# cxjyxxme/deep-online-video-stabilization

Hardware: AMD Instinct MI355X
Metric: stabilized frames/sec (720p, before_ch=31) (higher is better)
Workload: dtype f32 (bf16x3 split MFMA, f32 accumulate); 1 GPU; BASELINE.json configs[1]: v2_93 net, 1280x720, 1 stream(s)/GPU, batch=1 per stream, 13-ch stack from a 32-deep ring (lags 1,2,4,8,16,32; --before-ch 31 ignored as in the reference), ResNet-v2-50 regressor + 4x4 multi-grid warp + feedback; one independent stream set per GPU (replicas only); height=720, width=1280, streams_per_gpu=1, refine=1, operand_mode=4, launches_per_frame=64, hip_graph=True

## Files before the change

deep-online-video-stabilization_amd/csrc/conv.h:

```cpp
#pragma once
#include "common.h"

struct ConvArgs {
    const float* x;
    const float* w;
    float* y;
    const float* bias;
    const float* in_scale;
    const float* in_shift;
    const float* residual;
    const float* out_scale;
    const float* out_shift;
    const float* out_floor;
    float* partial;
    int N, H, W, Cin, Ho, Wo, Cout, KH, KW, stride, pad;
    int up;
    int res_H, res_W, res_stride;
    int relu_out;
    int x_ld, res_ld;
    int M, K;
    int splitk, steps_per_split;
    int cin_real;
    unsigned div_hw_mul, div_hw_shift, div_w_mul, div_w_shift;
    int rowrun;
    int in_scale_expected;
    int xcd_swizzle;
};

size_t conv_plan(ConvArgs& a);
struct Prof;
int conv_launch(const ConvArgs& a, hipStream_t st, Prof* prof = nullptr, int bf16_operands = 0, const float* w_img = nullptr,
                bool lowk_ring = false);

enum ConvFamily {
    CONV_IGEMM,
    CONV_RING,
    CONV_RING_KG,
    CONV_RING_PRO,
    CONV_PACKED,
    CONV_PACKED_KG2,
    CONV_ASTAT,
    CONV_PATCH
};
struct ConvRoute {
    int family;
    int tile, bk, nbuf;
    int mode;
    int operand;
    int kg, pro;
    int reduce;
    int prof_kind;
    int astat_bm;
    int patch_cfg;
};
ConvRoute conv_route(const ConvArgs& a, int operand_mode, bool has_image, bool bound, bool lowk_ring = false );
const char* conv_prof_kind_name(int kind);
size_t conv_weight_image_floats(int Cout, int K);
int launch_weight_split_image(const float* w, int Cout, int K, float* img, hipStream_t st);
struct WeightImageTable { long w_off[64], img_off[64], tprefix[65]; int Cout[64], K[64]; int n; };
void weight_image_table_add(WeightImageTable& t, long w_off, long img_off, int Cout, int K);
int launch_weight_split_images(const float* w_base, float* img_base, const WeightImageTable& t, hipStream_t st);
int conv_reduce_launches(const ConvArgs& a, int operand_mode = 0);

struct ConvPair { int m_tower, x_tower_floats ; long dx, dy, dres, dscale; };
bool conv_pair_supported(const ConvArgs& a);
int conv_launch_pair(const ConvArgs& a, const ConvPair& pr, hipStream_t st, Prof* prof = nullptr,
                     const float* w_img = nullptr );

bool conv_b2b_supported(const ConvArgs& c2, const ConvArgs& c3);
int conv_b2b_launch(const ConvArgs& c2, const ConvArgs& c3, hipStream_t st, Prof* prof = nullptr);

static inline void sn_fastdiv_make(unsigned d, unsigned& mul, unsigned& shift) {
    unsigned l = 0;
    while ((1ull << l) < d) ++l;
    mul = (unsigned)((((1ull << l) - d) << 32) / d + 1);
    shift = l;
}
#ifdef __HIPCC__
__device__ __forceinline__ int sn_fastdiv(int n, unsigned mul, unsigned shift) {
    return (int)((__umulhi(mul, (unsigned)n) + (unsigned)n) >> shift);
}
#endif
```

deep-online-video-stabilization_amd/csrc/conv.hip:

```cpp
#include "conv.h"
#include "prof.h"
#include <climits>
#include <cstdio>
#include <cstdlib>
#include <algorithm>
#include <string>
#include <vector>

#include "conv_kernel.h"
#include "conv_ring_kernel.h"
#include "conv_astat_kernel.h"
#include "conv_patch_kernel.h"
#include "conv_b2b_kernel.h"

template <int PAIR>
__device__ __forceinline__ void conv_splitk_reduce_body(const ConvArgs& p, const ConvPair& pr) {
    const size_t q = (size_t)blockIdx.x * 256 + threadIdx.x;
    const int c4n = p.Cout / 4;
    if (q >= (size_t)p.M * c4n) return;
    const int m = (int)(q / c4n);
    const int n = (int)(q - (size_t)m * c4n) * 4;
    const bool t1 = PAIR && m >= pr.m_tower;
    const size_t slab = (size_t)p.M * p.Cout;
    const float* src = p.partial + (size_t)m * p.Cout + n;
    float4 s = *reinterpret_cast<const float4*>(src);
    for (int z = 1; z < p.splitk; ++z) {
        const float4 t = *reinterpret_cast<const float4*>(src + z * slab);
        s.x += t.x; s.y += t.y; s.z += t.z; s.w += t.w;
    }
    if (p.bias != nullptr) {
        const float4 b = *reinterpret_cast<const float4*>(p.bias + n);
        s.x += b.x; s.y += b.y; s.z += b.z; s.w += b.w;
    }
    if (p.residual != nullptr) {
        size_t ri;
        if (p.res_stride == 1 && p.res_H == p.Ho && p.res_W == p.Wo) {
            ri = (size_t)m * p.res_ld + n;
        } else {
            const int img = sn_fastdiv(m, p.div_hw_mul, p.div_hw_shift);
            const int rr = m - img * (p.Ho * p.Wo);
            const int oy = sn_fastdiv(rr, p.div_w_mul, p.div_w_shift), ox = rr - oy * p.Wo;
            ri = (((size_t)img * p.res_H + oy * p.res_stride) * p.res_W + ox * p.res_stride) * p.res_ld + n;
        }
        const float4 t = *reinterpret_cast<const float4*>(p.residual + (t1 ? pr.dres : 0) + ri);
        s.x += t.x; s.y += t.y; s.z += t.z; s.w += t.w;
    }
    if (p.out_scale != nullptr) {
        const float4 a = *reinterpret_cast<const float4*>(p.out_scale + n), b = *reinterpret_cast<const float4*>(p.out_shift + n);
        s.x = __builtin_fmaf(s.x, a.x, b.x); s.y = __builtin_fmaf(s.y, a.y, b.y);
        s.z = __builtin_fmaf(s.z, a.z, b.z); s.w = __builtin_fmaf(s.w, a.w, b.w);
    }
    if (p.out_scale != nullptr && p.out_floor != nullptr) {
        const float4 f = *reinterpret_cast<const float4*>(p.out_floor + n);
        s.x = fmaxf(s.x, f.x); s.y = fmaxf(s.y, f.y); s.z = fmaxf(s.z, f.z); s.w = fmaxf(s.w, f.w);
    } else if (p.relu_out) {
        s.x = fmaxf(s.x, 0.f); s.y = fmaxf(s.y, 0.f); s.z = fmaxf(s.z, 0.f); s.w = fmaxf(s.w, 0.f);
    }
    *reinterpret_cast<float4*>(p.y + (t1 ? pr.dy : 0) + (size_t)m * p.Cout + n) = s;
}
__global__ __launch_bounds__(256) void conv_splitk_reduce_kernel(const ConvArgs p) {
    conv_splitk_reduce_body<0>(p, ConvPair{});
}
__global__ __launch_bounds__(256) void conv_splitk_reduce_pair_kernel(const ConvArgs p, const ConvPair pr) {
    conv_splitk_reduce_body<1>(p, pr);
}

enum TileId { T128x128 = 0, T128x64 = 1, T64x64 = 2 };

static void tile_dims(int t, int& bm, int& bn) {
    bm = (t == T64x64) ? 64 : 128;
    bn = (t == T128x128) ? 128 : 64;
}

static int env_int(const char* name, int dflt) {
    const char* v = getenv(name);
    return v ? atoi(v) : dflt;
}

struct ConvSwitches {
    int tile = env_int("STABNET_CONV_TILE", -1), splitk = env_int("STABNET_CONV_SPLITK", -1);
    int bk16 = env_int("STABNET_CONV_BK16", 0);
    int nbuf = env_int("STABNET_CONV_NBUF", 0);
    int tuning_table = env_int("STABNET_CONV_TUNING_TABLE", 1);
    int split_below = env_int("STABNET_CONV_SPLIT_BELOW", 400), split_target = env_int("STABNET_CONV_SPLIT_TARGET", 448);
    int xcd = env_int("STABNET_CONV_XCD", 1);
    int ring = env_int("STABNET_CONV_RING", 1), ring_wgs_per_cu = env_int("STABNET_CONV_RING_WGS_PER_CU", 3);
    int lowk_igemm = env_int("STABNET_CONV_LOWK_IGEMM", 1);
    int ring_pro = env_int("STABNET_CONV_RING_PRO", 1);
    int kgroups = env_int("STABNET_CONV_KGROUPS", 1), kgroups_pro = env_int("STABNET_CONV_KGROUPS_PRO", 1);
    int packed_kg2 = env_int("STABNET_CONV_PACKED_KG2", 1), packed_kg3 = env_int("STABNET_CONV_PACKED_KG3", 1);
    int packed_pro = env_int("STABNET_CONV_PACKED_PRO", 1);
    int packed_wgs_per_cu = env_int("STABNET_CONV_PACKED_WGS_PER_CU", 2);
    int astat = env_int("STABNET_CONV_ASTAT", 1), astat_min_m = env_int("STABNET_CONV_ASTAT_MIN_M", 0);
    int astat_min_cout = env_int("STABNET_CONV_ASTAT_MIN_COUT", 256);
    int patch = env_int("STABNET_CONV_PATCH", 1), patch_min_m = env_int("STABNET_CONV_PATCH_MIN_M", 0);
    int patch_cfg = env_int("STABNET_CONV_PATCH_CFG", 0);
    int b2b = env_int("STABNET_CONV_B2B", 1), b2b_wgs_per_cu = env_int("STABNET_CONV_B2B_WGS_PER_CU", 2);
};
static const ConvSwitches& sw() {
    static const ConvSwitches s;
    return s;
}

static int g_force_tile = -2, g_force_split = -1;
static int force_tile() { return g_force_tile == -2 ? sw().tile : g_force_tile; }
static int force_split() { return g_force_tile == -2 ? sw().splitk : g_force_split; }

static int conv_bk(const ConvArgs& a) { return (a.rowrun || (a.Cin % 32 == 0 && !sw().bk16)) ? 32 : 16; }
static int conv_total_steps(const ConvArgs& a) {
    if (a.rowrun) return a.KH * cdiv(a.KW * a.Cin, 32);
    return a.KH * a.KW * (a.Cin / conv_bk(a));
}

struct TuneEntry { int M, Cout, K, KH, ring, splitk; };
#include "conv_tuning_table.h"
#include "conv_tuning_table_packed.h"
static int g_tuning_profile = 0;
static std::vector<TuneEntry> g_tuning_runtime;

static int tuning_lookup(int M, int Cout, int K, int KH, int ring) {
    for (const TuneEntry& e : g_tuning_runtime)
        if (e.M == M && e.Cout == Cout && e.K == K && e.KH == KH && e.ring == ring) return e.splitk;
    if (sw().tuning_table && g_tuning_profile == 1)
        for (const TuneEntry& e : g_tuning_packed)
            if (e.M == M && e.Cout == Cout && e.K == K && e.KH == KH && e.ring == ring) return e.splitk;
    if (sw().tuning_table)
        for (const TuneEntry& e : g_tuning_builtin)
            if (e.M == M && e.Cout == Cout && e.K == K && e.KH == KH && e.ring == ring) return e.splitk;
    return 0;
}

static int pick_tile(const ConvArgs& a, int& splitk) {
    if (force_tile() >= 0) {
        const int steps0 = conv_total_steps(a);
        splitk = force_split() > 0 ? std::min(force_split(), steps0) : 1;
        return force_tile();
    }
    const int total_steps = conv_total_steps(a);
    const long blocks = (long)cdiv(a.M, 64) * cdiv(a.Cout, 64);
    const bool ring_path = a.rowrun || (a.in_scale_expected == 0 && a.up == 1 && a.Cin % 32 == 0);
    int s = tuning_lookup(a.M, a.Cout, a.K, a.KH, ring_path ? 1 : 0);
    const int thr = sw().split_below, target = sw().split_target;
    if (s > 0) {
        s = std::min(s, std::max(1, total_steps / 2));
    } else if (blocks < thr && a.Cout % 4 == 0) {
        s = (int)((target + blocks / 2) / blocks);
        s = std::min(s, std::max(1, total_steps / 8));
        s = std::min(s, 32);
    } else {
        s = 1;
    }
    splitk = std::max(1, s);
    return T64x64;
}

size_t conv_plan(ConvArgs& a) {
    a.xcd_swizzle = sw().xcd;
    a.M = a.N * a.Ho * a.Wo;
    a.K = a.rowrun ? a.KH * 32 * cdiv(a.KW * a.Cin, 32) : a.KH * a.KW * a.Cin;
    if (a.x_ld == 0) a.x_ld = a.Cin;
    if (a.res_ld == 0) a.res_ld = a.Cout;
    sn_fastdiv_make((unsigned)(a.Ho * a.Wo), a.div_hw_mul, a.div_hw_shift);
    sn_fastdiv_make((unsigned)a.Wo, a.div_w_mul, a.div_w_shift);
    int splitk = 1;
    (void)pick_tile(a, splitk);
    const int total_steps = conv_total_steps(a);
    a.steps_per_split = cdiv(total_steps, splitk);
    a.splitk = cdiv(total_steps, a.steps_per_split);
    return a.splitk > 1 ? (size_t)a.splitk * a.M * a.Cout * sizeof(float) : 0;
}

static void igemm_variant(const ConvArgs& a, int bm, int bn, int bk, int mode, int operand, int& nbuf_out, int& bf16_out) {
    const int nbuf = sw().nbuf;
    bf16_out = (bm == 64 && bn == 64 && bk == 32) ? operand : 0;
    const bool one_stage = nbuf == 1 || (nbuf == 0 && mode == 0 && bm == 64 && bn == 64 && a.M >= 32768);
    nbuf_out = (bf16_out != 1 && one_stage) ? 1 : 2;
}

static bool ring_eligible(const ConvArgs& a, int tile, bool has_prologue, bool lowk_ring = false) {
    if (a.rowrun) return true;
    if (!lowk_ring && sw().lowk_igemm && a.KH == 1 && a.KW == 1 && a.Cin == 64 && a.x_ld == a.Cin && a.out_floor == nullptr) return false;
    return sw().ring && tile == T64x64 && !has_prologue && a.up == 1 && a.Cin % 32 == 0 && !sw().bk16;
}

static bool ring_pro_vectors_ok(const ConvArgs& a) {
    if (a.in_scale == nullptr || a.in_shift == nullptr) return true;
    const long d = (long)(a.in_shift - a.in_scale);
    return d >= 0 && d < (1L << 30);
}
static bool ring_pro_geometry(const ConvArgs& a, int operand, bool has_prologue) {
    return sw().ring_pro && sw().ring && operand != 1 && !sw().bk16 && has_prologue && a.KH == 1 && a.KW == 1 && a.stride == 1 && a.pad == 0 &&
           a.up == 1 && a.Cin % 32 == 0 && !a.rowrun && a.x_ld == a.Cin;
}
static bool ring_pro_eligible(const ConvArgs& a, int operand) {
    return ring_pro_geometry(a, operand, a.in_scale != nullptr) && a.out_scale == nullptr && a.out_floor == nullptr && ring_pro_vectors_ok(a);
}

static int conv_kgroups(const ConvArgs& a, int operand, bool ring, bool has_prologue) {
    if (!sw().kgroups || a.splitk < 2 || operand == 1) return 1;
    if (a.steps_per_split * a.splitk != conv_total_steps(a)) return 1;
    if (ring && a.splitk == 3 && !a.rowrun) return 3;
    if (sw().kgroups_pro && !ring && a.splitk == 2 && ring_pro_geometry(a, operand, has_prologue) && ring_pro_vectors_ok(a)) return 2;
    return 1;
}

struct PatchForm { int ph, pw, wr, ns; };
static const PatchForm g_patch_forms[] = {{8, 8, 1, 3}, {8, 8, 2, 3}};
constexpr int SN_PATCH_FORMS = 2;
constexpr size_t SN_PATCH_LDS_MAX = 160 * 1024;
static int patch_cfg(const ConvArgs& a) {
    auto fits = [&](int cfg) { return sn_patch_lds_bytes(g_patch_forms[cfg - 1].ph, g_patch_forms[cfg - 1].pw, a.Cin) <= SN_PATCH_LDS_MAX; };
    const int forced = sw().patch_cfg;
    if (forced >= 1 && forced <= SN_PATCH_FORMS) return fits(forced) ? forced : 0;
    const int cfg = a.Cout <= 64 ? 1 : 2;
    return fits(cfg) ? cfg : 0;
}

static int route_prof_kind(const ConvRoute& r) {
    switch (r.family) {
        case CONV_IGEMM:
            return PK_KERNEL_CONV_BASE + r.mode * 6 + r.tile * 2 + (r.bk == 32 ? 1 : 0) + (r.nbuf == 1 ? 18 : 0) + 36 * r.operand;
        case CONV_PACKED: return PK_KERNEL_CONV_PACKED + (r.pro ? 3 : r.mode);
        case CONV_PACKED_KG2: return PK_KERNEL_CONV_PACKED + (r.pro ? 6 : 4 + r.mode);
        case CONV_ASTAT: return PK_KERNEL_CONV_ASTAT;
        case CONV_PATCH: return PK_KERNEL_CONV_PATCH + r.patch_cfg - 1;
        default: break;
    }
    const int split = r.operand >= 2 ? PK_KERNEL_CONV_SPLIT + 8 * (r.operand - 2) : 0;
    if (r.family == CONV_RING) return split ? split + r.mode : PK_KERNEL_CONV_RING + r.mode + (r.operand ? 3 : 0);
    if (r.family == CONV_RING_PRO) return split ? split + 5 : PK_KERNEL_CONV_KG + 2;
    if (r.kg == 2) return split ? split + 6 : PK_KERNEL_CONV_KG + 3;
    return split ? split + 3 + r.mode : PK_KERNEL_CONV_KG + r.mode;
}

ConvRoute conv_route(const ConvArgs& a, int operand_mode, bool has_image, bool bound, bool lowk_ring) {
    const ConvSwitches& s = sw();
    const bool image = operand_mode == 4 && has_image;
    const int op = operand_mode == 4 ? 0 : operand_mode;
    int splitk_unused = 1;
    const int t = pick_tile(a, splitk_unused);
    const bool t64 = t == T64x64, bk32 = conv_bk(a) == 32;
    const bool has_pro = bound ? a.in_scale != nullptr : a.in_scale_expected != 0;
    const bool ring = ring_eligible(a, t, has_pro, lowk_ring && image);
    const bool slabs = !bound || a.splitk == 1 || a.partial != nullptr;
    int kg = t64 ? conv_kgroups(a, op, ring, has_pro) : 1;
    if (image && s.packed_kg3 && ring && kg == 3 && a.K % 32 == 0 && slabs) kg = 1;
    const bool pro = kg == 1 && !ring && t64 && bk32 && (bound ? ring_pro_eligible(a, op) : ring_pro_geometry(a, op, has_pro));
    const bool packed_pro = image && s.packed_pro && !ring && t64 && bk32 && ring_pro_geometry(a, op, has_pro) &&
                            (!bound || a.out_floor == nullptr)  && ring_pro_vectors_ok(a) && slabs;
    if (packed_pro) kg = 1;
    const bool packed = (image && ring && kg == 1 && a.K % 32 == 0) || packed_pro;
    const bool packed_kg2 = packed && s.packed_kg2 && a.splitk == 2 && !a.rowrun && a.steps_per_split * 2 == conv_total_steps(a);
    if (packed_kg2) kg = 2;
    const int astat_min_m = s.astat_min_m > 0 ? s.astat_min_m : ((long)a.Cout * a.K >= 128 * 1024 ? 2048 : 8192);
    const bool astat = packed && !packed_pro && !packed_kg2 && kg == 1 && a.splitk == 1 && s.astat && !lowk_ring && !a.rowrun &&
                       a.KH == 1 && a.KW == 1 && a.stride == 1 && a.pad == 0 && a.up == 1 && a.K <= 256 && a.Cout >= s.astat_min_cout &&
                       a.M >= astat_min_m;
    const int patch_form = patch_cfg(a);
    const bool patch = packed && !packed_pro && ((kg == 1 && a.splitk == 1) || packed_kg2) && s.patch && !lowk_ring && !a.rowrun &&
                       a.KH == 3 && a.KW == 3 && a.stride == 1 && a.pad == 1 && a.up == 1 && a.Cin % 32 == 0 && patch_form != 0 &&
                       a.M >= (s.patch_min_m > 0 ? s.patch_min_m : 12288);

    ConvRoute r{};
    r.tile = t;
    r.bk = bk32 ? 32 : 16;
    r.mode = (a.up > 1 || a.rowrun) ? 2 : (a.pad == 0 ? 0 : 1);
    r.operand = op;
    r.kg = kg;
    r.reduce = (a.splitk > 1 && kg == 1) ? 1 : 0;
    if (astat) {
        r.family = CONV_ASTAT;
        r.operand = 4;
        r.astat_bm = 32;
    } else if (patch) {
        r.family = CONV_PATCH;
        r.operand = 4;
        r.patch_cfg = patch_form;
    } else if (packed) {
        r.family = packed_kg2 ? CONV_PACKED_KG2 : CONV_PACKED;
        r.operand = 4;
        r.pro = packed_pro ? 1 : 0;
    } else if (pro) {
        r.family = CONV_RING_PRO;
        r.pro = 1;
    } else if (kg > 1) {
        r.family = CONV_RING_KG;
        r.pro = kg == 2 ? 1 : 0;
    } else if (ring) {
        r.family = CONV_RING;
    } else {
        int bm, bn;
        tile_dims(t, bm, bn);
        r.family = CONV_IGEMM;
        igemm_variant(a, bm, bn, r.bk, r.mode, op, r.nbuf, r.operand);
    }
    r.prof_kind = route_prof_kind(r);
    return r;
}

int conv_reduce_launches(const ConvArgs& a, int operand_mode) {
    return a.splitk < 2 ? 0 : conv_route(a, operand_mode, operand_mode == 4, false).reduce;
}

const char* conv_prof_kind_name(int kind) {
    static const std::vector<std::string> names = [] {
        std::vector<std::string> v(PK_KERNEL_CONV_BASE + 144);
        char buf[96];
        auto ring = [&](int family, int mode, int operand, int kg, int pro) {
            ConvRoute r{};
            r.family = family; r.mode = mode; r.operand = operand; r.kg = kg; r.pro = pro;
            snprintf(buf, sizeof(buf), "conv_ring_f32_kernel<%d, %d, %d, %d>", mode, operand, kg, pro);
            v[route_prof_kind(r)] = buf;
        };
        for (int operand = 0; operand < 4; ++operand) {
            for (int mode = 0; mode < 3; ++mode) ring(CONV_RING, mode, operand, 1, 0);
            if (operand == 1) continue;
            ring(CONV_RING_KG, 0, operand, 3, 0); ring(CONV_RING_KG, 1, operand, 3, 0);
            ring(CONV_RING_PRO, 0, operand, 1, 1); ring(CONV_RING_KG, 0, operand, 2, 1);
        }
        for (int mode = 0; mode < 3; ++mode) ring(CONV_PACKED, mode, 4, 1, 0);
        ring(CONV_PACKED, 0, 4, 1, 1);
        ring(CONV_PACKED_KG2, 0, 4, 2, 0); ring(CONV_PACKED_KG2, 1, 4, 2, 0); ring(CONV_PACKED_KG2, 0, 4, 2, 1);
        {
            ConvRoute r{};
            r.family = CONV_ASTAT; r.astat_bm = 32;
            snprintf(buf, sizeof(buf), "conv_astat_f32_kernel<%d>", r.astat_bm);
            v[route_prof_kind(r)] = buf;
        }
        for (int cfg = 1; cfg <= SN_PATCH_FORMS; ++cfg) {
            ConvRoute r{};
            r.family = CONV_PATCH; r.patch_cfg = cfg;
            const PatchForm& f = g_patch_forms[cfg - 1];
            snprintf(buf, sizeof(buf), "conv_patch_f32_kernel<%d, %d, %d, %d>", f.ph, f.pw, f.wr, f.ns);
            v[route_prof_kind(r)] = buf;
        }
        for (int i = 0; i < 144; ++i) {
            ConvRoute r{};
            r.family = CONV_IGEMM;
            r.operand = i / 36; r.nbuf = 2 - i / 18 % 2; r.mode = i / 6 % 3; r.tile = i / 2 % 3; r.bk = (i & 1) ? 32 : 16;
            int bm, bn;
            tile_dims(r.tile, bm, bn);
            snprintf(buf, sizeof(buf), "conv_igemm_f32_kernel<%d, %d, %d, %d, %d, %d, %d, %d>", bm, bn, r.bk, bm / 2, bn / 2, r.mode, r.nbuf, r.operand);
            v[route_prof_kind(r)] = buf;
        }
        for (int i = 0; i < 4; ++i) {
            snprintf(buf, sizeof(buf), "conv_igemm_f32_pair_kernel<64, 64, %d, 32, 32, %d>", (i & 1) ? 32 : 16, i / 2);
            v[PK_KERNEL_CONV_PAIR + i] = buf;
        }
        v[PK_KERNEL_CONV_B2B] = "conv_b2b_f32_kernel<2>";
        v[PK_KERNEL_CONV_B2B + 1] = "conv_b2b_f32_kernel<4>";
        return v;
    }();
    return (kind >= 0 && kind < (int)names.size() && !names[kind].empty()) ? names[kind].c_str() : nullptr;
}

template <int BM, int BN, int BK, int WM, int WN, int MODE, int NBUF, int BF16 = 0>
static int launch_one_nb(const ConvArgs& a, hipStream_t st) {
    constexpr size_t lds_op = NBUF * (size_t)(BM + BN) * (BK + 4) * sizeof(float);
    constexpr size_t lds_epi = 4 * (size_t)SN_EPI_WAVE_BYTES;
    constexpr size_t lds = lds_op > lds_epi ? lds_op : lds_epi;
    static bool configured = false;
    auto kern = conv_igemm_f32_kernel<BM, BN, BK, WM, WN, MODE, NBUF, BF16>;
    if (!configured) {
        if (lds > 64 * 1024) {
            hipError_t e = hipFuncSetAttribute(reinterpret_cast<const void*>(kern),
                                               hipFuncAttributeMaxDynamicSharedMemorySize, (int)lds);
            if (e != hipSuccess) {
                stabnet_set_error("conv: hipFuncSetAttribute(%zu B LDS) failed: %s", lds, hipGetErrorString(e));
                return STABNET_ERR_LAUNCH;
            }
        }
        configured = true;
    }
    dim3 grid(cdiv(a.M, BM), cdiv(a.Cout, BN), a.splitk);
    kern<<<grid, 256, lds, st>>>(a);
    SN_LAUNCH_CHECK("conv_igemm_f32_kernel");
    return STABNET_OK;
}

template <int BM, int BN, int BK, int WM, int WN, int MODE>
static int launch_one_t(const ConvRoute& r, const ConvArgs& a, hipStream_t st) {
    if constexpr (BM == 64 && BN == 64 && BK == 32) {
        if (r.operand == 1) return launch_one_nb<BM, BN, BK, WM, WN, MODE, 2, 1>(a, st);
        else if (r.operand == 2) return r.nbuf == 1 ? launch_one_nb<BM, BN, BK, WM, WN, MODE, 1, 2>(a, st) : launch_one_nb<BM, BN, BK, WM, WN, MODE, 2, 2>(a, st);
        else if (r.operand == 3) return r.nbuf == 1 ? launch_one_nb<BM, BN, BK, WM, WN, MODE, 1, 3>(a, st) : launch_one_nb<BM, BN, BK, WM, WN, MODE, 2, 3>(a, st);
    }
    return r.nbuf == 1 ? launch_one_nb<BM, BN, BK, WM, WN, MODE, 1>(a, st) : launch_one_nb<BM, BN, BK, WM, WN, MODE, 2>(a, st);
}

template <int BM, int BN, int BK, int WM, int WN>
static int launch_one(const ConvRoute& r, const ConvArgs& a, hipStream_t st) {
    if (r.mode == 2) return launch_one_t<BM, BN, BK, WM, WN, 2>(r, a, st);
    if (r.mode == 0) return launch_one_t<BM, BN, BK, WM, WN, 0>(r, a, st);
    return launch_one_t<BM, BN, BK, WM, WN, 1>(r, a, st);
}

static int launch_igemm(const ConvRoute& r, const ConvArgs& a, hipStream_t st) {
    if (r.bk == 32) {
        if (r.tile == T128x128) return launch_one<128, 128, 32, 64, 64>(r, a, st);
        if (r.tile == T128x64) return launch_one<128, 64, 32, 64, 32>(r, a, st);
        return launch_one<64, 64, 32, 32, 32>(r, a, st);
    }
    if (r.tile == T128x128) return launch_one<128, 128, 16, 64, 64>(r, a, st);
    if (r.tile == T128x64) return launch_one<128, 64, 16, 64, 32>(r, a, st);
    return launch_one<64, 64, 16, 32, 32>(r, a, st);
}

static int device_cus(int& cus) {
    static int cached = 0;
    if (cached == 0) {
        int dev = 0, n = 0;
        if (hipGetDevice(&dev) != hipSuccess || hipDeviceGetAttribute(&n, hipDeviceAttributeMultiprocessorCount, dev) != hipSuccess || n <= 0) {
            stabnet_set_error("conv: cannot read the CU count");
            return STABNET_ERR_LAUNCH;
        }
        cached = n;
    }
    cus = cached;
// ... 12 lines not shown
    if constexpr (B != 1) {
        if (key == 11) { conv_ring_f32_kernel<0, B, 1, 1><<<grid, 256, 0, st>>>(a); return true; }
        if (key == 21) { conv_ring_f32_kernel<0, B, 2, 1><<<grid, 512, 0, st>>>(a); return true; }
    }
    if constexpr (B == 0 || B == 2 || B == 3) {
        if (key == 30) { conv_ring_f32_kernel<0, B, 3><<<grid, 768, 0, st>>>(a); return true; }
        if (key == 130) { conv_ring_f32_kernel<1, B, 3><<<grid, 768, 0, st>>>(a); return true; }
    }
    if constexpr (B == 4) {
        if (key == 20) { conv_ring_f32_kernel<0, B, 2, 0><<<grid, 512, 0, st>>>(a); return true; }
        if (key == 120) { conv_ring_f32_kernel<1, B, 2, 0><<<grid, 512, 0, st>>>(a); return true; }
    }
    return false;
}

static int launch_ring_route(const ConvRoute& r, const ConvArgs& a, hipStream_t st) {
    int cus = 0;
    if (const int rc = device_cus(cus)) return rc;
    const int per_cu = r.kg > 1 ? 1 : (r.operand == 4 ? sw().packed_wgs_per_cu : sw().ring_wgs_per_cu);
    const long ntiles = (long)cdiv(a.M, 64) * cdiv(a.Cout, 64) * (r.kg > 1 ? 1 : a.splitk);
    const int grid = (int)std::min<long>(ntiles, (long)per_cu * usable_cus(cus));
    bool ok = false;
    switch (r.operand) {
        case 0: ok = launch_ring_operand<0>(r, a, grid, st); break;
        case 1: ok = launch_ring_operand<1>(r, a, grid, st); break;
        case 2: ok = launch_ring_operand<2>(r, a, grid, st); break;
        case 3: ok = launch_ring_operand<3>(r, a, grid, st); break;
        case 4: ok = launch_ring_operand<4>(r, a, grid, st); break;
        default: break;
    }
    SN_REQUIRE(ok, "conv: no conv_ring_f32_kernel<%d, %d, %d, %d>", r.mode, r.operand, r.kg, r.pro);
    SN_LAUNCH_CHECK("conv_ring_f32_kernel");
    return STABNET_OK;
}

static int launch_astat(const ConvRoute& r, const ConvArgs& a, hipStream_t st) {
    int cus = 0;
    if (const int rc = device_cus(cus)) return rc;
    const int bm = r.astat_bm;
    SN_REQUIRE(bm == 32 && a.K % 32 == 0 && (size_t)bm * a.K * 6 <= (size_t)SN_ASTAT_A_BYTES && a.splitk == 1,
               "conv: the A-stationary kernel takes BM %d x K %d without a K split only if the planes fit %d bytes", bm, a.K, SN_ASTAT_A_BYTES);
    const int mtiles = cdiv(a.M, bm), nblk = 2 * cdiv(a.Cout, 64);
    int groups = (int)std::min<long>(cdiv(nblk, 4), std::max<long>(1, 2L * usable_cus(cus) / mtiles));
    groups = cdiv(nblk, 4 * cdiv(cdiv(nblk, groups), 4));
    const dim3 grid(mtiles, groups);
    conv_astat_f32_kernel<32><<<grid, 256, 0, st>>>(a);
    SN_LAUNCH_CHECK("conv_astat_f32_kernel");
    return STABNET_OK;
}

template <int PH, int PW, int WR, int NS>
static int launch_patch_one(const ConvArgs& a, int cus, hipStream_t st) {
    const size_t lds = sn_patch_lds_bytes(PH, PW, a.Cin);
    auto kern = conv_patch_f32_kernel<PH, PW, WR, NS>;
    static size_t configured = 64 * 1024;
    if (lds > configured) {
        hipError_t e = hipFuncSetAttribute(reinterpret_cast<const void*>(kern), hipFuncAttributeMaxDynamicSharedMemorySize, (int)SN_PATCH_LDS_MAX);
        if (e != hipSuccess) {
            stabnet_set_error("conv: hipFuncSetAttribute(%zu B LDS) failed: %s", SN_PATCH_LDS_MAX, hipGetErrorString(e));
            return STABNET_ERR_LAUNCH;
        }
        configured = SN_PATCH_LDS_MAX;
    }
    constexpr int cs = 4 / ((PH / 4) * (PW / 8) / WR);
    const int mtiles = a.N * cdiv(a.Ho, PH) * cdiv(a.Wo, PW), nblk = 2 * cdiv(a.Cout, 64);
    const long slots = (long)std::min<size_t>(WR >= 4 ? 1 : 2, SN_PATCH_LDS_MAX / lds) * usable_cus(cus);
    int groups = (int)std::min<long>(cdiv(nblk, cs), std::max<long>(1, slots / mtiles));
    groups = cdiv(nblk, cs * cdiv(cdiv(nblk, groups), cs));
    const dim3 grid(mtiles, groups);
    kern<<<grid, 256, lds, st>>>(a);
    SN_LAUNCH_CHECK("conv_patch_f32_kernel");
    return STABNET_OK;
}
static int launch_patch(const ConvRoute& r, const ConvArgs& a, hipStream_t st) {
    int cus = 0;
    if (const int rc = device_cus(cus)) return rc;
    SN_REQUIRE(a.KH == 3 && a.KW == 3 && a.stride == 1 && a.pad == 1 && a.up == 1 && a.Cin % 32 == 0 &&
                   (a.splitk == 1 || (a.splitk == 2 && a.steps_per_split * 2 == conv_total_steps(a))) && a.Ho == a.H && a.Wo == a.W && r.patch_cfg >= 1 &&
                   r.patch_cfg <= SN_PATCH_FORMS &&
                   sn_patch_lds_bytes(g_patch_forms[r.patch_cfg - 1].ph, g_patch_forms[r.patch_cfg - 1].pw, a.Cin) <= SN_PATCH_LDS_MAX,
               "conv: the patch-stationary kernel takes 3x3 / pad 1 / stride 1 over Cin %d (a multiple of 32) without a K split or with two equal K halves only if the planes fit %zu bytes",
               a.Cin, SN_PATCH_LDS_MAX);
    return r.patch_cfg == 1 ? launch_patch_one<8, 8, 1, 3>(a, cus, st) : launch_patch_one<8, 8, 2, 3>(a, cus, st);
}

size_t conv_weight_image_floats(int Cout, int K) { return (size_t)cdiv(Cout, 64) * (size_t)(K / 32) * 3072; }

__device__ __forceinline__ unsigned weight_split_head(float& x0, float& x1) {
    const float top = __builtin_bit_cast(float, 0x7F7F0000u), fmax = __builtin_bit_cast(float, 0x7F7FFFFFu);
    const float h0 = (fabsf(x0) > top && fabsf(x0) <= fmax) ? copysignf(top, x0) : x0;
    const float h1 = (fabsf(x1) > top && fabsf(x1) <= fmax) ? copysignf(top, x1) : x1;
    const unsigned p = sn_pack_bf16(h0, h1);
    x0 = sn_sub_f32(x0, __builtin_bit_cast(float, p << 16));
    x1 = sn_sub_f32(x1, __builtin_bit_cast(float, p & 0xffff0000u));
    return p;
}
__device__ __forceinline__ SnSplit3 weight_split3(const f32x4 x) {
    float a = x.x, b = x.y, c = x.z, d = x.w;
    typedef unsigned u32x2 __attribute__((ext_vector_type(2)));
    u32x2 h, m, l;
    h.x = weight_split_head(a, b); h.y = weight_split_head(c, d);
    m.x = sn_split_level(a, b); m.y = sn_split_level(c, d);
    l.x = sn_pack_bf16(a, b); l.y = sn_pack_bf16(c, d);
    SnSplit3 s;
    s.h = __builtin_bit_cast(sn_bf16x4, h); s.m = __builtin_bit_cast(sn_bf16x4, m); s.l = __builtin_bit_cast(sn_bf16x4, l);
    return s;
}

__device__ __forceinline__ void weight_split_image_thread(const float* __restrict__ w, int Cout, int K, uint4* __restrict__ img, long i) {
    const int steps = K / 32;
    const int lane = (int)(i & 63), j = (int)((i >> 6) & 1), wn = (int)((i >> 7) & 1);
    const long ts = i >> 8;
    const int ks = (int)(ts % steps), nt = (int)(ts / steps);
    const int n = nt * 64 + wn * 32 + (lane & 31), g = lane >> 5;
    f32x4 lo = {0.f, 0.f, 0.f, 0.f}, hi = lo;
    if (n < Cout) {
        const float* r = w + (size_t)n * K + ks * 32 + 16 * j + 4 * g;
        lo = *reinterpret_cast<const f32x4*>(r);
        hi = *reinterpret_cast<const f32x4*>(r + 8);
    }
    const SnSplit3 a = weight_split3(lo), b = weight_split3(hi);
    uint4* out = img + ts * 768 + (size_t)(wn * 6 + j) * 64 + lane;
    out[0] = __builtin_bit_cast(uint4, SN_CAT8(a.h, b.h));
    out[2 * 64] = __builtin_bit_cast(uint4, SN_CAT8(a.m, b.m));
    out[4 * 64] = __builtin_bit_cast(uint4, SN_CAT8(a.l, b.l));
}

__global__ __launch_bounds__(256) void weight_split_image_kernel(const float* __restrict__ w, int Cout, int K, uint4* __restrict__ img) {
    const long i = (long)blockIdx.x * 256 + threadIdx.x;
    if (i >= (long)((Cout + 63) / 64) * (K / 32) * 256) return;
    weight_split_image_thread(w, Cout, K, img, i);
}

__global__ __launch_bounds__(256) void weight_split_images_kernel(const float* __restrict__ w_base, float* __restrict__ img_base, const WeightImageTable t) {
    const long i = (long)blockIdx.x * 256 + threadIdx.x;
    if (i >= t.tprefix[t.n]) return;
    int e = 0;
    while (i >= t.tprefix[e + 1]) ++e;
    weight_split_image_thread(w_base + t.w_off[e], t.Cout[e], t.K[e], reinterpret_cast<uint4*>(img_base + t.img_off[e]), i - t.tprefix[e]);
}

void weight_image_table_add(WeightImageTable& t, long w_off, long img_off, int Cout, int K) {
    if (t.n == 0) t.tprefix[0] = 0;
    t.w_off[t.n] = w_off; t.img_off[t.n] = img_off; t.Cout[t.n] = Cout; t.K[t.n] = K;
    t.tprefix[t.n + 1] = t.tprefix[t.n] + (long)cdiv(Cout, 64) * (K / 32) * 256;
    ++t.n;
}

int launch_weight_split_images(const float* w_base, float* img_base, const WeightImageTable& t, hipStream_t st) {
    if (t.n == 0) return STABNET_OK;
    SN_REQUIRE(w_base && img_base && t.n <= 64, "weight images: bad table");
    weight_split_images_kernel<<<(unsigned)(t.tprefix[t.n] >> 8), 256, 0, st>>>(w_base, img_base, t);
    SN_LAUNCH_CHECK("weight_split_images_kernel");
    return STABNET_OK;
}

int launch_weight_split_image(const float* w, int Cout, int K, float* img, hipStream_t st) {
    SN_REQUIRE(w && img && Cout > 0 && K > 0 && K % 32 == 0, "weight image: K=%d must be a multiple of 32", K);
    const long total = (long)cdiv(Cout, 64) * (K / 32) * 256;
    weight_split_image_kernel<<<cdiv(total, 256), 256, 0, st>>>(w, Cout, K, reinterpret_cast<uint4*>(img));
    SN_LAUNCH_CHECK("weight_split_image_kernel");
    return STABNET_OK;
}

int conv_launch(const ConvArgs& a, hipStream_t st, Prof* prof, int bf16_operands, const float* w_img, bool lowk_ring) {
    SN_REQUIRE(a.rowrun || a.Cin % 16 == 0, "conv: Cin=%d must be a multiple of 16 (pad the channels)", a.Cin);
    SN_REQUIRE(!a.rowrun || (a.in_scale == nullptr && a.up == 1 && a.KH <= 8 && cdiv(a.KW * a.Cin, 32) <= 4),
               "conv: row-run operand needs no prologue, KH <= 8 and KW*Cin <= 128");
    SN_REQUIRE(a.Cout % 4 == 0, "conv: Cout=%d must be a multiple of 4", a.Cout);
    SN_REQUIRE(a.splitk >= 1 && a.steps_per_split >= 1 && a.div_hw_mul != 0, "conv: conv_plan() not called");
    SN_REQUIRE(a.splitk == 1 || a.partial != nullptr, "conv: split-K needs a workspace");
    const ConvRoute r = conv_route(a, bf16_operands, w_img != nullptr, true, lowk_ring);
    SN_REQUIRE(r.family != CONV_IGEMM || a.x_ld == a.Cin, "conv: a strided input (x_ld %d != Cin %d) needs the ring kernel", a.x_ld, a.Cin);
    g_last_launch_kind = r.prof_kind;
    const bool rec = prof != nullptr && prof->begin(st);
    int rc;
    switch (r.family) {
        case CONV_IGEMM: rc = launch_igemm(r, a, st); break;
        case CONV_PACKED:
        case CONV_PACKED_KG2: {
            ConvArgs b = a;
            b.w = w_img;
            rc = launch_ring_route(r, b, st);
            break;
        }
        case CONV_ASTAT: {
            ConvArgs b = a;
            b.w = w_img;
            rc = launch_astat(r, b, st);
            break;
        }
        case CONV_PATCH: {
            ConvArgs b = a;
            b.w = w_img;
            rc = launch_patch(r, b, st);
            break;
        }
        default: rc = launch_ring_route(r, a, st); break;
    }
    if (rec) prof->end(st, r.prof_kind, 2.0 * a.M * (double)(a.KH * a.KW * (a.cin_real ? a.cin_real : a.Cin)) * a.Cout,
                       4.0 * ((double)a.N * a.H * a.W * a.Cin + (double)a.K * a.Cout + (double)a.M * a.Cout * (r.reduce ? a.splitk : 1) +
                              ((a.residual != nullptr && !r.reduce) ? (double)a.M * a.Cout : 0.0)),
                       a.M, a.Cout, a.K, a.splitk);
    if (rc) return rc;
    if (r.reduce) {
        const size_t q = (size_t)a.M * (a.Cout / 4);
        const bool rec2 = prof != nullptr && prof->begin(st);
        conv_splitk_reduce_kernel<<<cdiv((long)q, 256), 256, 0, st>>>(a);
        if (rec2) prof->end(st, PK_KERNEL_SPLITK_REDUCE, 0.0, 4.0 * (double)a.M * a.Cout * (a.splitk + 1 + (a.residual != nullptr ? 1 : 0)));
        SN_LAUNCH_CHECK("conv_splitk_reduce_kernel");
    }
    return STABNET_OK;
}

bool conv_pair_supported(const ConvArgs& a) {
    int splitk_unused = 1;
    const int t = pick_tile(a, splitk_unused);
    const bool pro = a.in_scale != nullptr || a.in_scale_expected;
    return t == T64x64 && !ring_eligible(a, t, pro) && a.up == 1 && !a.rowrun && (a.x_ld == 0 || a.x_ld == a.Cin);
}

template <int BK, int MODE>
static int launch_pair_one(const ConvArgs& a, const ConvPair& pr, hipStream_t st) {
    constexpr size_t lds = 2 * (size_t)(64 + 64) * (BK + 4) * sizeof(float);
    static_assert(lds >= 4 * (size_t)SN_EPI_WAVE_BYTES && lds <= 64 * 1024, "LDS of the 64x64 tile");
    dim3 grid(cdiv(a.M, 64), cdiv(a.Cout, 64), a.splitk);
    conv_igemm_f32_pair_kernel<64, 64, BK, 32, 32, MODE><<<grid, 256, lds, st>>>(a, pr);
    SN_LAUNCH_CHECK("conv_igemm_f32_pair_kernel");
    return STABNET_OK;
}

int conv_launch_pair(const ConvArgs& a, const ConvPair& pr, hipStream_t st, Prof* prof, const float* w_img) {
    SN_REQUIRE(a.Cin % 16 == 0 && a.Cout % 4 == 0, "conv pair: Cin %% 16 and Cout %% 4 must be 0");
    SN_REQUIRE(a.splitk >= 1 && a.steps_per_split >= 1 && a.div_hw_mul != 0, "conv pair: conv_plan() not called");
    SN_REQUIRE(a.splitk == 1 || a.partial != nullptr, "conv pair: split-K needs a workspace");
    SN_REQUIRE(conv_pair_supported(a), "conv pair: the plan of this shape is not the 64x64 register-staged launch");
    SN_REQUIRE(pr.m_tower > 0 && pr.m_tower % 64 == 0 && a.M == 2 * pr.m_tower, "conv pair: tower rows %d must be a multiple of 64 (M %d)",
               pr.m_tower, a.M);
    const bool bk32 = conv_bk(a) == 32;
    const int mode = a.pad == 0 ? 0 : 1;
    const bool pro = bk32 && ring_pro_eligible(a, 0) && pr.dx == pr.dscale - (long)pr.m_tower * a.Cin && pr.dy == pr.dscale - (long)pr.m_tower * a.Cout &&
                     (a.residual == nullptr || pr.dres == pr.dscale - (long)(a.N / 2) * a.res_H * a.res_W * a.res_ld);
    const bool packed = pro && w_img != nullptr && a.K % 32 == 0 && a.splitk == 1;
    ConvRoute r{};
    r.family = packed ? CONV_PACKED : CONV_RING_PRO;
    r.operand = packed ? 4 : 0;
    r.kg = r.pro = 1;
    g_last_launch_kind = pro ? route_prof_kind(r) : PK_KERNEL_CONV_PAIR + mode * 2 + (bk32 ? 1 : 0);
    const bool rec = prof != nullptr && prof->begin(st);
    int rc;
    if (pro) {
        ConvArgs b = a;
        b.out_floor = reinterpret_cast<const float*>((size_t)pr.dscale);
        if (packed) b.w = w_img;
        rc = launch_ring_route(r, b, st);
    } else if (bk32) {
        rc = mode == 0 ? launch_pair_one<32, 0>(a, pr, st) : launch_pair_one<32, 1>(a, pr, st);
    } else {
        rc = mode == 0 ? launch_pair_one<16, 0>(a, pr, st) : launch_pair_one<16, 1>(a, pr, st);
    }
    if (rec) prof->end(st, pro ? route_prof_kind(r) : PK_KERNEL_CONV_PAIR + mode * 2 + (bk32 ? 1 : 0), 2.0 * a.M * (double)(a.KH * a.KW * (a.cin_real ? a.cin_real : a.Cin)) * a.Cout,
                       4.0 * ((double)a.N * a.H * a.W * a.Cin + (double)a.K * a.Cout + (double)a.M * a.Cout * a.splitk),
                       a.M, a.Cout, a.K, a.splitk);
    if (rc) return rc;
    if (a.splitk > 1) {
        const size_t q = (size_t)a.M * (a.Cout / 4);
        const bool rec2 = prof != nullptr && prof->begin(st);
        conv_splitk_reduce_pair_kernel<<<cdiv((long)q, 256), 256, 0, st>>>(a, pr);
        if (rec2) prof->end(st, PK_KERNEL_SPLITK_REDUCE, 0.0, 4.0 * (double)a.M * a.Cout * (a.splitk + 1));
        SN_LAUNCH_CHECK("conv_splitk_reduce_pair_kernel");
    }
    return STABNET_OK;
}

bool conv_b2b_supported(const ConvArgs& c2, const ConvArgs& c3) {
    const bool g2 = c2.KH == 3 && c2.KW == 3 && c2.pad == 1 && c2.up == 1 && !c2.rowrun && (c2.stride == 1 || c2.stride == 2) &&
                    c2.Cin == c2.Cout && (c2.Cout == 64 || c2.Cout == 128) && c2.in_scale_expected == 0 && c2.in_scale == nullptr;
    const bool g3 = c3.KH == 1 && c3.KW == 1 && c3.pad == 0 && c3.stride == 1 && c3.up == 1 && !c3.rowrun && c3.Cin == c2.Cout &&
// ... 230 lines not shown
```

deep-online-video-stabilization_amd/csrc/prof.h:

```cpp
#pragma once
#include <vector>
#include "common.h"

enum {
    PK_KERNEL_PAD = 1, PK_KERNEL_POOL = 2, PK_KERNEL_GAP = 3, PK_KERNEL_FC = 4, PK_KERNEL_MESH = 5,
    PK_KERNEL_WARP = 6, PK_KERNEL_ASSEMBLE = 7, PK_KERNEL_PUSH = 8, PK_KERNEL_SPLITK_REDUCE = 9, PK_KERNEL_WGRAD = 10, PK_KERNEL_HEAD = 20,
    PK_KERNEL_MJPEG_TRANSFORM = 30, PK_KERNEL_MJPEG_ENTROPY = 31, PK_KERNEL_MJPEG_LAYOUT = 32, PK_KERNEL_MJPEG_GATHER = 33 ,
    PK_KERNEL_INGEST_GREY_ROWS = 34, PK_KERNEL_INGEST_GREY_COLS = 35, PK_KERNEL_INGEST_COLOUR = 36 ,
    PK_KERNEL_MAP_SHRINK = 37, PK_KERNEL_REMAP_SRC = 38, PK_KERNEL_REMAP_SRC4 = 39 ,
    PK_KERNEL_REMAP_WIN = 60, PK_KERNEL_REMAP_WIN4 = 61 ,
    PK_KERNEL_REMAP_WIN_DEV = 62, PK_KERNEL_REMAP_WIN4_DEV = 63 ,
    PK_KERNEL_REMAP_I420 = 59 ,
    PK_KERNEL_REMAP_CUBIC = 250 ,
    PK_KERNEL_REMAP_I420_CUBIC = 256 ,
    PK_KERNEL_MJPEGD_PLANES = 257 ,
    PK_KERNEL_MJPEG_TRANSFORM_PLANAR = 258 ,
    PK_KERNEL_TF_GET_IMG = 64,
    PK_KERNEL_TVL1_STEP = 57, PK_KERNEL_TVL1_FUSED = 58 ,
    PK_KERNEL_TVL1_DOWN = 65, PK_KERNEL_TVL1_GRAD = 66, PK_KERNEL_TVL1_WARP = 67, PK_KERNEL_TVL1_UP = 68, PK_KERNEL_TVL1_MAP = 69 ,
    PK_KERNEL_KLT_DETECT = 26, PK_KERNEL_KLT_TRACK = 27, PK_KERNEL_KLT_FINISH = 28 ,
    PK_KERNEL_HOMFIT = 29 ,
    PK_KERNEL_WGRAD_SAME = 11 ,
    PK_KERNEL_CONV_PAIR = 80 , PK_KERNEL_CONV_KG = 84 , PK_KERNEL_CONV_RING = 90 ,
    PK_KERNEL_CONV_PACKED = 70 ,
    PK_KERNEL_CONV_ASTAT = 77 ,
    PK_KERNEL_CONV_PATCH = 24 ,
    PK_KERNEL_CONV_B2B = 96 ,
    PK_KERNEL_CONV_SPLIT = 40 ,
    PK_KERNEL_CONV_BASE = 100
};

struct Prof {
    std::vector<hipEvent_t> ev;
    std::vector<int> kind;
    std::vector<double> flops, bytes;
    std::vector<int> shape;
    int cap = 0, n = 0;
    bool begin(hipStream_t st) {
        if (n >= cap) return false;
        (void)hipEventRecord(ev[2 * n], st);
        return true;
    }
    void end(hipStream_t st, int k, double f, double b, int sm = 0, int sn = 0, int sk = 0, int ss = 0) {
        (void)hipEventRecord(ev[2 * n + 1], st);
        kind[n] = k; flops[n] = f; bytes[n] = b;
        shape[4 * n] = sm; shape[4 * n + 1] = sn; shape[4 * n + 2] = sk; shape[4 * n + 3] = ss;
        ++n;
    }
};
```

Measured before the change: 691.3 frames/s.

## Add row-segment stem conv kernel staging input rows in LDS as bf16x3 planes

Adds a dedicated kernel for the large row-run stem convolution. It loads one padded input row segment covering 128 output pixels into LDS once per kernel row, splits it into three bf16 planes, and double-buffers the next row while MFMA runs over the overlapping windows. The aim is to cut redundant global reads of overlapping strided patches that the generic packed path does for the wide stem. It adds a new routing condition with shape restrictions and some ablation macros, so only layers that match the constraints use it.

```diff
diff --git a/deep-online-video-stabilization_amd/csrc/conv.h b/deep-online-video-stabilization_amd/csrc/conv.h
--- a/deep-online-video-stabilization_amd/csrc/conv.h
+++ b/deep-online-video-stabilization_amd/csrc/conv.h
@@ -40,7 +40,8 @@
     CONV_PACKED,
     CONV_PACKED_KG2,
     CONV_ASTAT,
-    CONV_PATCH
+    CONV_PATCH,
+    CONV_STEM
 };
 struct ConvRoute {
     int family;
diff --git a/deep-online-video-stabilization_amd/csrc/conv.hip b/deep-online-video-stabilization_amd/csrc/conv.hip
--- a/deep-online-video-stabilization_amd/csrc/conv.hip
+++ b/deep-online-video-stabilization_amd/csrc/conv.hip
@@ -11,6 +11,7 @@
 #include "conv_ring_kernel.h"
 #include "conv_astat_kernel.h"
 #include "conv_patch_kernel.h"
+#include "conv_stem_kernel.h"
 #include "conv_b2b_kernel.h"
 
 template <int PAIR>
@@ -95,6 +96,7 @@
     int astat_min_cout = env_int("STABNET_CONV_ASTAT_MIN_COUT", 256);
     int patch = env_int("STABNET_CONV_PATCH", 1), patch_min_m = env_int("STABNET_CONV_PATCH_MIN_M", 0);
     int patch_cfg = env_int("STABNET_CONV_PATCH_CFG", 0);
+    int stem = env_int("STABNET_CONV_STEM", 1), stem_min_m = env_int("STABNET_CONV_STEM_MIN_M", 0);
     int b2b = env_int("STABNET_CONV_B2B", 1), b2b_wgs_per_cu = env_int("STABNET_CONV_B2B_WGS_PER_CU", 2);
 };
 static const ConvSwitches& sw() {
@@ -224,6 +226,7 @@
         case CONV_PACKED_KG2: return PK_KERNEL_CONV_PACKED + (r.pro ? 6 : 4 + r.mode);
         case CONV_ASTAT: return PK_KERNEL_CONV_ASTAT;
         case CONV_PATCH: return PK_KERNEL_CONV_PATCH + r.patch_cfg - 1;
+        case CONV_STEM: return PK_KERNEL_CONV_STEM;
         default: break;
     }
     const int split = r.operand >= 2 ? PK_KERNEL_CONV_SPLIT + 8 * (r.operand - 2) : 0;
@@ -260,6 +263,10 @@
     const bool patch = packed && !packed_pro && ((kg == 1 && a.splitk == 1) || packed_kg2) && s.patch && !lowk_ring && !a.rowrun &&
                        a.KH == 3 && a.KW == 3 && a.stride == 1 && a.pad == 1 && a.up == 1 && a.Cin % 32 == 0 && patch_form != 0 &&
                        a.M >= (s.patch_min_m > 0 ? s.patch_min_m : 12288);
+    const bool stem = packed && !packed_pro && !packed_kg2 && kg == 1 && a.splitk == 1 && s.stem && !lowk_ring && a.rowrun && a.up == 1 &&
+                      a.KH <= 8 && a.KW * a.Cin <= 128 && a.K == a.KH * 32 * SN_STEM_RS && (a.stride * a.Cin) % 2 == 0 &&
+                      a.stride * a.Cin * (SN_STEM_PIX - 1) + 32 * SN_STEM_RS <= sn_stem_seg(SN_STEM_RS, SN_STEM_PIX) &&
+                      a.M >= (s.stem_min_m > 0 ? s.stem_min_m : 65536);
 
     ConvRoute r{};
     r.tile = t;
@@ -276,6 +283,9 @@
         r.family = CONV_PATCH;
         r.operand = 4;
         r.patch_cfg = patch_form;
+    } else if (stem) {
+        r.family = CONV_STEM;
+        r.operand = 4;
     } else if (packed) {
         r.family = packed_kg2 ? CONV_PACKED_KG2 : CONV_PACKED;
         r.operand = 4;
@@ -334,6 +344,8 @@
             snprintf(buf, sizeof(buf), "conv_patch_f32_kernel<%d, %d, %d, %d>", f.ph, f.pw, f.wr, f.ns);
             v[route_prof_kind(r)] = buf;
         }
+        snprintf(buf, sizeof(buf), "conv_stem_f32_kernel<%d, %d, %d>", SN_STEM_RS, SN_STEM_WR, SN_STEM_PIX);
+        v[PK_KERNEL_CONV_STEM] = buf;
         for (int i = 0; i < 144; ++i) {
             ConvRoute r{};
             r.family = CONV_IGEMM;
@@ -512,6 +524,17 @@
                "conv: the patch-stationary kernel takes 3x3 / pad 1 / stride 1 over Cin %d (a multiple of 32) without a K split or with two equal K halves only if the planes fit %zu bytes",
                a.Cin, SN_PATCH_LDS_MAX);
     return r.patch_cfg == 1 ? launch_patch_one<8, 8, 1, 3>(a, cus, st) : launch_patch_one<8, 8, 2, 3>(a, cus, st);
+}
+
+static int launch_stem(const ConvArgs& a, hipStream_t st) {
+    SN_REQUIRE(a.rowrun && a.splitk == 1 && a.up == 1 && a.in_scale == nullptr && a.K == a.KH * 32 * SN_STEM_RS && (a.stride * a.Cin) % 2 == 0 &&
+                   a.stride * a.Cin * (SN_STEM_PIX - 1) + 32 * SN_STEM_RS <= sn_stem_seg(SN_STEM_RS, SN_STEM_PIX),
+               "conv: the stem kernel takes row-run launches of %d-float runs without a K split whose 128-pixel segment fits %d elements (stride %d, Cin %d)",
+               32 * SN_STEM_RS, sn_stem_seg(SN_STEM_RS, SN_STEM_PIX), a.stride, a.Cin);
+    const dim3 grid(a.N * a.Ho * cdiv(a.Wo, SN_STEM_PIX), cdiv(a.Cout, 64));
+    conv_stem_f32_kernel<SN_STEM_RS, SN_STEM_WR, SN_STEM_PIX><<<grid, sn_stem_threads(SN_STEM_WR, SN_STEM_PIX), 0, st>>>(a);
+    SN_LAUNCH_CHECK("conv_stem_f32_kernel");
+    return STABNET_OK;
 }
 
 size_t conv_weight_image_floats(int Cout, int K) { return (size_t)cdiv(Cout, 64) * (size_t)(K / 32) * 3072; }
@@ -624,6 +647,12 @@
             ConvArgs b = a;
             b.w = w_img;
             rc = launch_patch(r, b, st);
+            break;
+        }
+        case CONV_STEM: {
+            ConvArgs b = a;
+            b.w = w_img;
+            rc = launch_stem(b, st);
             break;
         }
         default: rc = launch_ring_route(r, a, st); break;
diff --git a/deep-online-video-stabilization_amd/csrc/conv_stem_kernel.h b/deep-online-video-stabilization_amd/csrc/conv_stem_kernel.h
--- /dev/null
+++ b/deep-online-video-stabilization_amd/csrc/conv_stem_kernel.h
@@ -0,0 +1,152 @@
+#pragma once
+#include "conv_patch_kernel.h"
+
+#ifndef STEM_ABLATE
+#define STEM_ABLATE 0
+#endif
+
+#ifndef STEM_WR
+#define STEM_WR 2
+#define STEM_PIX 128
+#endif
+constexpr int SN_STEM_RS = 3, SN_STEM_WR = STEM_WR, SN_STEM_PIX = STEM_PIX;
+constexpr int SN_STEM_PITCH = 26;
+constexpr int sn_stem_seg(int rs, int pix) { return (SN_STEM_PITCH * (pix - 1) + 32 * rs + 7) / 8 * 8; }
+constexpr int sn_stem_threads(int wr, int pix) { return 64 * 2 * (pix / (32 * wr)); }
+
+template <int RS , int WR ,
+          int PIX >
+__global__ __launch_bounds__(sn_stem_threads(WR, PIX), WR >= 4 ? 2 : 3) void conv_stem_f32_kernel(const ConvArgs p) {
+    static_assert(RS >= 2 && RS <= 4, "runs of 64 to 128 floats");
+    static_assert(PIX % (32 * WR) == 0, "whole row units");
+    constexpr int NT = sn_stem_threads(WR, PIX), NWAVES = NT / 64;
+    constexpr int SEG = sn_stem_seg(RS, PIX), PLANE_BYTES = SEG * 2, BUF_BYTES = 3 * PLANE_BYTES;
+    constexpr int NQ = (SEG / 4 + NT - 1) / NT;
+    static_assert(BUF_BYTES % 16 == 0 && BUF_BYTES >= NWAVES * SN_EPI_WAVE_BYTES, "the epilogue scratch overlays one buffer");
+    typedef unsigned u32x2 __attribute__((ext_vector_type(2)));
+    typedef unsigned u32x2a4 __attribute__((ext_vector_type(2), aligned(4)));
+    typedef float f32x4a4 __attribute__((ext_vector_type(4), aligned(4)));
+    __shared__ __attribute__((aligned(16))) unsigned char stem_lds[2 * BUF_BYTES];
+
+    const int tid = threadIdx.x, lane = tid & 63, wave = __builtin_amdgcn_readfirstlane(tid >> 6);
+    const ConvTile tile = conv_tile_of_block(p);
+    const int tiles_x = (p.Wo + PIX - 1) / PIX, tiles_img = tiles_x * p.Ho;
+    const int img = tile.mt / tiles_img, t_in = tile.mt - img * tiles_img;
+    const int oy = t_in / tiles_x, ox0 = (t_in - oy * tiles_x) * PIX;
+    const int npix = min(PIX, p.Wo - ox0);
+    const int pitch = p.stride * p.Cin;
+    const int nload = pitch * (npix - 1) + 32 * RS;
+    const int row_floats = (p.W + 2 * p.pad) * p.Cin;
+    const float* const seg0 = p.x + ((size_t)(img * (p.H + 2 * p.pad) + oy * p.stride) * (p.W + 2 * p.pad) + ox0 * p.stride) * p.Cin;
+
+    f32x4 sv[NQ];
+    auto seg_load = [&](const float* s) {
+#pragma unroll
+        for (int i = 0; i < NQ; ++i) {
+            if (!(STEM_ABLATE & 1)) sv[i] = *reinterpret_cast<const f32x4a4*>(s + min(4 * (tid + NT * i), nload - 4));
+            else sv[i] = f32x4{(float)tid, (float)i, (float)(size_t)s, 1.f};
+        }
+        __builtin_amdgcn_sched_barrier(0);
+    };
+    auto seg_store = [&](unsigned char* buf) {
+        if (STEM_ABLATE & 16) return;
+#pragma unroll
+        for (int i = 0; i < NQ; ++i) {
+            const int qi = tid + NT * i;
+            if (4 * qi < nload) {
+                const bool moved = 4 * qi > nload - 4;
+                float a = moved ? sv[i].z : sv[i].x, b = moved ? sv[i].w : sv[i].y, c = moved ? 0.f : sv[i].z, d = moved ? 0.f : sv[i].w;
+                u32x2 h, m, l;
+                h.x = sn_split_level(a, b); h.y = sn_split_level(c, d);
+                m.x = sn_split_level(a, b); m.y = sn_split_level(c, d);
+                l.x = sn_pack_bf16(a, b); l.y = sn_pack_bf16(c, d);
+                *reinterpret_cast<u32x2*>(buf + 8 * qi) = h;
+                *reinterpret_cast<u32x2*>(buf + PLANE_BYTES + 8 * qi) = m;
+                *reinterpret_cast<u32x2*>(buf + 2 * PLANE_BYTES + 8 * qi) = l;
+            }
+        }
+    };
+
+    const int unit = wave >> 1, wn = wave & 1;
+    const bool active = unit * 32 * WR < npix;
+    const int m0 = (img * p.Ho + oy) * p.Wo + ox0;
+    int mrow[WR][4];
+    unsigned a_off[WR];
+#pragma unroll
+    for (int i = 0; i < WR; ++i) {
+        a_off[i] = (unsigned)(2 * pitch * (unit * 32 * WR + i * 32 + (lane & 31)) + 8 * (lane >> 5));
+#pragma unroll
+        for (int q = 0; q < 4; ++q) {
+            const int px = unit * 32 * WR + i * 32 + (lane >> 3) + 8 * q;
+            mrow[i][q] = px < npix ? m0 + px : -1;
+        }
+    }
+    const int steps = p.KH * RS;
+    const f32x4* lp = reinterpret_cast<const f32x4*>(p.w) + ((size_t)tile.nt * steps * 12 + wn * 6) * 64 + lane;
+    int l_step = 0;
+    auto load = [&](f32x4 (&dst)[6]) {
+        if ((STEM_ABLATE & 2) && l_step >= RS - 1) { ++l_step; return; }
+#pragma unroll
+        for (int i = 0; i < 6; ++i) dst[i] = lp[i * 64];
+        lp += l_step + 1 < steps ? 768 : 0;
+        ++l_step;
+        __builtin_amdgcn_sched_barrier(0);
+    };
+    f32x16 acc[WR][1];
+#pragma unroll
+    for (int i = 0; i < WR; ++i)
+#pragma unroll
+        for (int e = 0; e < 16; ++e) acc[i][0][e] = 0.f;
+    auto step = [&](const unsigned char* buf, int rs, const f32x4 (&B)[6]) {
+#pragma unroll
+        for (int j = 0; j < 2; ++j) {
+            SnPlanes A[WR];
+#pragma unroll
+            for (int i = 0; i < WR; ++i) {
+                const unsigned char* ap = buf + (a_off[i] + (unsigned)(32 * (2 * rs + j)));
+                const u32x2 h0 = *reinterpret_cast<const u32x2a4*>(ap), h1 = *reinterpret_cast<const u32x2a4*>(ap + 16);
+                const u32x2 m0_ = *reinterpret_cast<const u32x2a4*>(ap + PLANE_BYTES), m1 = *reinterpret_cast<const u32x2a4*>(ap + PLANE_BYTES + 16);
+                const u32x2 l0 = *reinterpret_cast<const u32x2a4*>(ap + 2 * PLANE_BYTES), l1 = *reinterpret_cast<const u32x2a4*>(ap + 2 * PLANE_BYTES + 16);
+                A[i].h = sn_u32x4{h0.x, h0.y, h1.x, h1.y};
+                A[i].m = sn_u32x4{m0_.x, m0_.y, m1.x, m1.y};
+                A[i].l = sn_u32x4{l0.x, l0.y, l1.x, l1.y};
+                if (STEM_ABLATE & 8) A[i].h = A[i].m = A[i].l = sn_u32x4{(unsigned)(size_t)ap, (unsigned)rs, (unsigned)lane, 1u};
+            }
+            const sn_bf16x8 bh = __builtin_bit_cast(sn_bf16x8, B[j]), bm = __builtin_bit_cast(sn_bf16x8, B[2 + j]), bl = __builtin_bit_cast(sn_bf16x8, B[4 + j]);
+#define SN_STEM_MFMA(ap_, b_)                                                                                                       \
+    _Pragma("unroll") for (int i = 0; i < WR; ++i)                                                                                  \
+        acc[i][0] = __builtin_amdgcn_mfma_f32_32x32x16_bf16(__builtin_bit_cast(sn_bf16x8, A[i].ap_), b_, acc[i][0], 0, 0, 0)
+            SN_STEM_MFMA(l, bh);
+            SN_STEM_MFMA(h, bl);
+            SN_STEM_MFMA(m, bm);
+            SN_STEM_MFMA(m, bh);
+            SN_STEM_MFMA(h, bm);
+            SN_STEM_MFMA(h, bh);
+#undef SN_STEM_MFMA
+        }
+    };
+
+    f32x4 B[RS][6];
+#pragma unroll
+    for (int s = 0; s < RS - 1; ++s) load(B[s]);
+    seg_load(seg0);
+    seg_store(stem_lds);
+    __syncthreads();
+    for (int kh = 0; kh < p.KH; ++kh) {
+        const bool more = kh + 1 < p.KH;
+        if (more) seg_load(seg0 + (size_t)(kh + 1) * row_floats);
+        const unsigned char* const cur = stem_lds + (kh & 1) * BUF_BYTES;
+#pragma unroll
+        for (int rs = 0; rs < RS; ++rs) {
+            load(B[(rs + RS - 1) % RS]);
+            if (active) step(cur, rs, B[rs]);
+        }
+        if (more) {
+            seg_store(stem_lds + ((kh + 1) & 1) * BUF_BYTES);
+            __syncthreads();
+        }
+    }
+    if (!active) return;
+    float* const scratch = reinterpret_cast<float*>(stem_lds + (p.KH & 1) * BUF_BYTES + wave * SN_EPI_WAVE_BYTES);
+    conv_patch_epilogue<WR>(acc, p, mrow, m0, tile.nt * 64 + wn * 32, lane, scratch);
+}
diff --git a/deep-online-video-stabilization_amd/csrc/prof.h b/deep-online-video-stabilization_amd/csrc/prof.h
--- a/deep-online-video-stabilization_amd/csrc/prof.h
+++ b/deep-online-video-stabilization_amd/csrc/prof.h
@@ -25,6 +25,7 @@
     PK_KERNEL_CONV_PACKED = 70 ,
     PK_KERNEL_CONV_ASTAT = 77 ,
     PK_KERNEL_CONV_PATCH = 24 ,
+    PK_KERNEL_CONV_STEM = 78 ,
     PK_KERNEL_CONV_B2B = 96 ,
     PK_KERNEL_CONV_SPLIT = 40 ,
     PK_KERNEL_CONV_BASE = 100
```

Result: no change. 693.1 frames/s, median of 6 (+0.3%).
